# atharris/basilisk_env

Measured on AMD Instinct MI355X. Metric: env steps/sec at 65k parallel spacecraft, 1/2/4/8 MI355X; HBM GB/s vs roofline, higher is better.
Workload: dtype f64; 1 GPU; BASELINE configs[2]: 65536 envs/GPU, J2 + 4 reaction wheels (pyramid) + nadir reward, f64, dt 0.1 s, K=1 RK4 sub-step(s)/env step, FSW every 10 (fsw_lag=nav_lag=1), synthetic PCG64(rank); envs_per_gpu=65536, substeps=1, scenario=bare, batch_stats=per-wave sums in the step launch; join on demand, kernel_fingerprint=2b375b0f4a16a217

## Files before the change

basilisk_env_amd/csrc/bsk_device.hpp:

```cpp
#pragma once
#include <hip/hip_runtime.h>
#include <stdint.h>

#include <type_traits>

#include "../../include/bskgpu.h"
#include "bsk_probes.hpp"

namespace bsk {

#define BSK_LIKELY(x) __builtin_expect(!!(x), 1)
#define BSK_UNLIKELY(x) __builtin_expect(!!(x), 0)

struct V3 {
    double x, y, z;
};
__device__ __forceinline__ V3 mk(double x, double y, double z) { return V3{x, y, z}; }
__device__ __forceinline__ V3 operator+(V3 a, V3 b) { return V3{a.x + b.x, a.y + b.y, a.z + b.z}; }
__device__ __forceinline__ V3 operator-(V3 a, V3 b) { return V3{a.x - b.x, a.y - b.y, a.z - b.z}; }
__device__ __forceinline__ V3 operator*(double s, V3 a) { return V3{s * a.x, s * a.y, s * a.z}; }
__device__ __forceinline__ double dot(V3 a, V3 b) { return fma(a.x, b.x, fma(a.y, b.y, a.z * b.z)); }
__device__ __forceinline__ V3 cross(V3 a, V3 b) {
    return V3{fma(a.y, b.z, -(a.z * b.y)), fma(a.z, b.x, -(a.x * b.z)), fma(a.x, b.y, -(a.y * b.x))};
}
// ... 141 lines not shown
    double mu_sun;
    double base_density;
    double inv_scale_height, inv_mass, rho_skip;
    int32_t desat, pad_;
};

struct PowerCfg {
    double nB[3];
    double kflux;
    double draw, cap;
    double req, rs_plus, rs_minus;
    double rsun;
    double sun_r0[3], sun_v[3];
};

struct SunGeom {
    V3 sun;
    double ism;
    double re_sf1, re_sf2;
    double tf1, tf2;
};

__device__ __forceinline__ SunGeom sun_setup(const PowerCfg& pc, double t0) {
    SunGeom g;
    g.sun = mk(fma(pc.sun_v[0], t0, pc.sun_r0[0]), fma(pc.sun_v[1], t0, pc.sun_r0[1]), fma(pc.sun_v[2], t0, pc.sun_r0[2]));
    g.ism = rsqrt_nr(dot(g.sun, g.sun));
    const double sf1 = pc.rs_plus * g.ism, sf2 = pc.rs_minus * g.ism;
    g.re_sf1 = pc.req * rcp_nr(sf1);
    g.re_sf2 = pc.req * rcp_nr(sf2);
    g.tf1 = sf1 * rsqrt_nr(fma(-sf1, sf1, 1.0));
    g.tf2 = sf2 * rsqrt_nr(fma(-sf2, sf2, 1.0));
    return g;
}

__device__ __forceinline__ double asin_small(double s) {
    const double z = s * s;
    return s * fma(z, fma(z, fma(z, fma(z, 35.0 / 1152.0, 15.0 / 336.0), 3.0 / 40.0), 1.0 / 6.0), 1.0);
}

__device__ __forceinline__ double asin_core(double z) {
    double p = 0.03187962140081284;
    p = fma(p, z, -0.016187392271599134);
    p = fma(p, z, 0.019513468251252167);
    p = fma(p, z, 0.0065293020047365695);
    p = fma(p, z, 0.012170138592391726);
    p = fma(p, z, 0.01388484282640208);
    p = fma(p, z, 0.01735977964134998);
    p = fma(p, z, 0.022371749733164054);
    p = fma(p, z, 0.03038195969768514);
    p = fma(p, z, 0.044642856805998936);
    p = fma(p, z, 0.07500000000385201);
    p = fma(p, z, 0.16666666666664942);
    return fma(p, z, 1.0);
}
__device__ __forceinline__ double asin01(double s) {
    const bool big = s > 0.5;
    const double z = big ? fma(-0.5, s, 0.5) : s * s;
    const double q = big ? sqrt_nr(z) : s;
    const double r = q * asin_core(z);
    return big ? fma(-2.0, r, 1.57079632679489661923) : r;
}
__device__ __forceinline__ double angle_xy(double x, double y, double a) {
    const double ia = rcp_nr(a), t = x * ia, sy = y * ia, at = fabs(t);
    const bool big = at > 0.5;
    const double z = big ? 0.5 * sy * sy * rcp_nr(1.0 + at) : t * t;
    const double q = big ? sqrt_nr(z) : at;
    const double r = q * asin_core(z);
    const double PI = 3.14159265358979323846;
    const double base = big ? (t > 0.0 ? 0.0 : PI) : 0.5 * PI;
    const double k = big ? (t > 0.0 ? 2.0 : -2.0) : (t > 0.0 ? -1.0 : 1.0);
    return fma(k, r, base);
}

__device__ __attribute__((noinline)) double percent_shadow_generic(double sa, double sb, double cc) {
    const double PI = 3.14159265358979323846;
    const double a = asin(sa), b = asin(sb), c = acos(cc);
    if (c < a - b) return 1.0 - (b * b) / (a * a);
    const double x = (c * c + a * a - b * b) / (2.0 * c), y = sqrt(fmax(a * a - x * x, 0.0));
    const double area = a * a * acos(x / a) + b * b * acos((c - x) / b) - c * y;
    return 1.0 - area / (PI * a * a);
}

__device__ __forceinline__ double percent_shadow(const PowerCfg& pc, V3 r_HB, V3 r, double r2) {
    const double nh2 = dot(r_HB, r_HB);
    const double inh = rsqrt_nr(nh2), ins = rsqrt_nr(r2);
    const double sa = fmin(pc.rsun * inh, 1.0), sb = fmin(pc.req * ins, 1.0);
    const double cc = fmax(fmin(-dot(r, r_HB) * inh * ins, 1.0), -1.0);
    const double ca = sqrt_nr(fma(-sa, sa, 1.0)), cb = sqrt_nr(fma(-sb, sb, 1.0));
    if (sb > sa && cc > fma(cb, ca, sb * sa)) return 0.0;
    if (cc <= fma(cb, ca, -(sb * sa))) return 1.0;
    const double PI = 3.14159265358979323846;
    if (sa < 0.03125 * sb) {
        const double a = asin_small(sa), b = asin01(sb);
        const double sc = sqrt_nr(fma(-cc, cc, 1.0));
        const double d = asin_small(fma(sc, cb, -(cc * sb)));
        const double c = b + d, a2 = a * a;
        const double x = fma(d, fma(2.0, b, d), a2) * rcp_nr(2.0 * c);
        const double y = sqrt_nr(fmax(fma(-x, x, a2), 0.0));
        const double th1 = angle_xy(x, y, a);
        const double w = y * rcp_nr(b), z = w * w;
        const double t2 = w * z * fma(z, fma(z, fma(z, 35.0 / 1152.0, 15.0 / 336.0), 3.0 / 40.0), 1.0 / 6.0);
        const double area = fma(a2, th1, fma(b * b, t2, -(d * y)));
        return 1.0 - area * rcp_nr(PI * a2);
    }
    return percent_shadow_generic(sa, sb, cc);
}

constexpr int PEN_CHUNK = 10;
constexpr int PEN_SLOTS = 30;
constexpr int PEN_QCAP = 192;
struct PowerLds {
    double g[PEN_SLOTS][64];
    double s[PEN_SLOTS][64];
    double sun[3][64];
    double qr[3][PEN_QCAP];
    int qown[PEN_QCAP];
    int qcount, pad_[3];
};
typedef PowerLds __attribute__((address_space(3))) * LdsP;

constexpr int PAIR_CHUNK = 10;
struct PairLds {
    double rr[2][3][PAIR_CHUNK][64];
    double rs[2][3][PAIR_CHUNK][64];
    double box[16][64];
    double sfac[PAIR_CHUNK][64];
    double sun[3][64];
    double lext[3][64];
    int qown[PAIR_CHUNK * 64];
    int qcount, pad_[3];
};
typedef PairLds __attribute__((address_space(3))) * PairP;

constexpr int PART_ALL = 0, PART_ROT = 1, PART_TRA = 2;

constexpr int TRI_SPIN_LIMIT = 1 << 20;
enum { BSK_DEVERR_TRI_EXCHANGE = 1, BSK_DEVERR_FORK_MAP = 2 };
struct TriX {
    double v[4][4][64];
    double s[4][3][64];
    int tv[4][64], ts[4][64];
    int err, pad0_;
    int pad_[4];
};
struct TriLds {
    PairLds p;
    TriX x;
};
typedef TriX __attribute__((address_space(3))) * TriXP;
typedef TriLds __attribute__((address_space(3))) * TriP;

struct HalvesLds {
    double rv[6][64];
    unsigned long long orbit;
    unsigned long long pad_;
};
typedef HalvesLds __attribute__((address_space(3))) * HalvesP;

__device__ __forceinline__ void tri_order() { asm volatile("" ::: "memory"); }
__device__ __forceinline__ void tri_st(double __attribute__((address_space(3))) * p, double v) {
    __hip_atomic_store((long long __attribute__((address_space(3)))*)p, __double_as_longlong(v), __ATOMIC_RELAXED, __HIP_MEMORY_SCOPE_WORKGROUP);
}
__device__ __forceinline__ double tri_ld(const double __attribute__((address_space(3))) * p) {
    return __longlong_as_double(__hip_atomic_load((long long __attribute__((address_space(3)))*)p, __ATOMIC_RELAXED, __HIP_MEMORY_SCOPE_WORKGROUP));
}
__device__ __forceinline__ void tri_sti(int __attribute__((address_space(3))) * p, int v) { __hip_atomic_store(p, v, __ATOMIC_RELAXED, __HIP_MEMORY_SCOPE_WORKGROUP); }
__device__ __forceinline__ int tri_ldi(int __attribute__((address_space(3))) * p) { return __hip_atomic_load(p, __ATOMIC_RELAXED, __HIP_MEMORY_SCOPE_WORKGROUP); }

struct TriPend {
    int tag;
    V3 a;
    double e;
};
template <int PART>
struct TriXch {
    TriXP X;
    int lane;
    int np, nc;
    bool dead;
    unsigned dbg_miss = 0, dbg_spin = 0;
    unsigned long long dbg_cyc = 0;
    template <bool EXTRA>
    __device__ __forceinline__ void publish(V3 a, double extra) {
        if constexpr (probe::TRI_NOPUBLISH && PART == PART_TRA) { ++np; return; }
        const int slot = np & 3;
        if constexpr (PART == PART_TRA) {
            tri_st(&X->v[slot][0][lane], a.x); tri_st(&X->v[slot][1][lane], a.y); tri_st(&X->v[slot][2][lane], a.z);
            if constexpr (EXTRA) tri_st(&X->v[slot][3][lane], extra);
            tri_order();
            tri_sti(&X->tv[slot][lane], np + 1);
        } else {
            tri_st(&X->s[slot][0][lane], a.x); tri_st(&X->s[slot][1][lane], a.y); tri_st(&X->s[slot][2][lane], a.z);
            tri_order();
            tri_sti(&X->ts[slot][lane], np + 1);
        }
        tri_order();
        ++np;
    }
    template <bool EXTRA>
    __device__ __forceinline__ TriPend prefetch() const {
        const int slot = nc & 3;
        TriPend f;
        f.e = 0.0;
        if constexpr (PART == PART_TRA) {
            f.tag = tri_ldi(&X->ts[slot][lane]);
            tri_order();
            f.a = mk(tri_ld(&X->s[slot][0][lane]), tri_ld(&X->s[slot][1][lane]), tri_ld(&X->s[slot][2][lane]));
        } else {
            f.tag = tri_ldi(&X->tv[slot][lane]);
            tri_order();
            f.a = mk(tri_ld(&X->v[slot][0][lane]), tri_ld(&X->v[slot][1][lane]), tri_ld(&X->v[slot][2][lane]));
            if constexpr (EXTRA) f.e = tri_ld(&X->v[slot][3][lane]);
        }
        return f;
    }
    template <bool EXTRA>
    __device__ __forceinline__ V3 finish(TriPend f, double& extra) {
        const int want = nc + 1;
        if (BSK_UNLIKELY(__builtin_amdgcn_ballot_w64(f.tag != want) != 0)) {
            if constexpr (probe::XCH_STATS) ++dbg_miss;
            const probe::Stamp c0 = probe::stamp<probe::XCH_STATS>();
            for (int spin = 0; !dead; ++spin) {
                f = prefetch<EXTRA>();
                if constexpr (probe::XCH_STATS) ++dbg_spin;
                if (__builtin_amdgcn_ballot_w64(f.tag != want) == 0) break;
                if (spin > TRI_SPIN_LIMIT) { dead = true; X->err = 1; }
            }
            probe::since<probe::XCH_STATS>(dbg_cyc, c0);
        }
        ++nc;
        if constexpr (EXTRA) extra = f.e;
        return f.a;
    }
};

struct KTab {
    double a, b, c, e;
};
template <int K>
__device__ __forceinline__ double fmac_k(double acc, double tab, double x) {
    static_assert(K >= 0 && K < 16, "row lane");
    asm volatile("v_fmac_f64_dpp %0, %1, %2 row_newbcast:%3 row_mask:0xf bank_mask:0xf" : "+v"(acc) : "v"(tab), "v"(x), "n"(K));
    return acc;
}
template <int K>
__device__ __forceinline__ double fmac_k_abs(double acc, double tab, double x) {
    asm volatile("v_fmac_f64_dpp %0, %1, |%2| row_newbcast:%3 row_mask:0xf bank_mask:0xf" : "+v"(acc) : "v"(tab), "v"(x), "n"(K));
    return acc;
}
template <int K>
__device__ __forceinline__ double fmac_k_neg(double acc, double tab, double x) {
    asm volatile("v_fmac_f64_dpp %0, %1, -%2 row_newbcast:%3 row_mask:0xf bank_mask:0xf" : "+v"(acc) : "v"(tab), "v"(x), "n"(K));
    return acc;
}
__device__ __forceinline__ double max0(double x) {
    double r;
    asm("v_max_f64 %0, %1, 0" : "=v"(r) : "v"(x));
    return r;
}
template <int K>
__device__ __forceinline__ double mul_k(double tab, double x) { return fmac_k<K>(0.0, tab, x); }
template <int K>
__device__ __forceinline__ double get_k(double tab) {
    double r;
    asm volatile("v_mov_b64_dpp %0, %1 row_newbcast:%2 row_mask:0xf bank_mask:0xf" : "=v"(r) : "v"(tab), "n"(K));
    return r;
}

__device__ __forceinline__ double atmosphere_exponent(const KTab& kt, double rm) {
    return fmac_k<KC_NIH>(get_k<KC_REQIH>(kt.c), kt.c, rm);
}
__device__ __forceinline__ double atmosphere_exp(const KTab& kt, double x) {
    const double n = __builtin_rint(mul_k<KC_LOG2E>(kt.c, x));
    const double te = kt.e;
    double r = fmac_k<KE_NLN2HI>(x, te, n);
    double t0 = get_k<KE_POLY + 0>(te), t1 = get_k<KE_POLY + 2>(te), t2 = get_k<KE_POLY + 4>(te), t3 = get_k<KE_POLY + 6>(te);
    r = fmac_k<KE_NLN2LO>(r, te, n);
    double t4 = get_k<KE_POLY + 8>(te), t5 = get_k<KE_POLY + 10>(te), t6 = get_k<KE_POLY + 12>(te);
    const double r2 = r * r;
    t0 = fmac_k<KE_POLY + 1>(t0, te, r); t1 = fmac_k<KE_POLY + 3>(t1, te, r); t2 = fmac_k<KE_POLY + 5>(t2, te, r);
    t3 = fmac_k<KE_POLY + 7>(t3, te, r); t4 = fmac_k<KE_POLY + 9>(t4, te, r); t5 = fmac_k<KE_POLY + 11>(t5, te, r);
    t6 = fmac_k<KE_POLY + 13>(t6, te, r);
    double p = fma(t6, r2, t5);
    p = fma(p, r2, t4);
    p = fma(p, r2, t3);
    p = fma(p, r2, t2);
    p = fma(p, r2, t1);
    p = fma(p, r2, t0);
    return ldexp(p, (int)n);
}
struct Atmo {
    double x, rho;
    __device__ __forceinline__ double clamped(const KTab& kt) const { return rho >= get_k<KC_RSKIP>(kt.c) ? rho : 0.0; }
    __device__ __forceinline__ double anchor(const KTab& kt, double rm) {
        x = atmosphere_exponent(kt, rm);
        rho = atmosphere_exp(kt, x);
        return clamped(kt);
    }
    __device__ __forceinline__ double advance(const KTab& kt, double rm) {
        const double xn = atmosphere_exponent(kt, rm);
        const double d = xn - x;
        x = xn;
        const double d2 = d * d;
        double a = fmac_k<KC_I120>(get_k<KC_I24>(kt.c), kt.c, d);
        double b = fmac_k<KC_I6>(0.5, kt.c, d);
        a = fmac_k<KC_I720>(a, kt.c, d2);
        b = fma(d2, a, b);
// ... 995 lines not shown
```

basilisk_env_amd/csrc/bsk_kernels.hip:

```cpp
#include "bsk_device.hpp"
#include "bsk_envstep.hpp"
#include "bsk_launch.hpp"

#include <atomic>
#include <cstddef>
#define __COMMA__ ,

namespace bsk {

__device__ __forceinline__ int uni(bool b) { return __builtin_amdgcn_readfirstlane(b ? 1 : 0); }
__device__ __forceinline__ double own_scalar(double x) {
    const unsigned long long u = __builtin_bit_cast(unsigned long long, x);
    const unsigned lo = __builtin_amdgcn_readfirstlane((unsigned)u), hi = __builtin_amdgcn_readfirstlane((unsigned)(u >> 32));
    return __builtin_bit_cast(double, ((unsigned long long)hi << 32) | lo);
}
__device__ __forceinline__ int uni_any(bool lane_cond) {
    const unsigned long long m = __builtin_amdgcn_ballot_w64(lane_cond);
    int r;
    asm volatile("s_cmp_lg_u64 %1, 0\n\ts_cselect_b32 %0, 1, 0" : "=s"(r) : "s"(m) : "scc");
    return r;
}

__device__ __forceinline__ int halves_fsw_due(int cnt_x, int nav_lag, int fsw_every) {
    return uni_any((cnt_x >> 20) == (nav_lag != 0 ? fsw_every - 1 : 0));
}

__device__ __forceinline__ int wave_min_uniform(int v) {
    const int first = __builtin_amdgcn_readfirstlane(v);
    if (__builtin_amdgcn_ballot_w64(v != first) == 0) return first;
#pragma unroll
    for (int off = 32; off > 0; off >>= 1) v = min(v, __shfl_xor(v, off, 64));
    return __builtin_amdgcn_readfirstlane(v);
}

constexpr int LDSS_WAVES = 3;
template <int GRAV, int NRW, bool DIAG, int FEAT, int SPLIT>
__global__ __launch_bounds__(256, (SPLIT == 5 || SPLIT == 4 || SPLIT == 2 || SPLIT == 3 || SPLIT == 6) ? 2 : (FEAT == FEAT_LDSS ? LDSS_WAVES : 1)) void step_kernel(const StepArgs<NRW, DIAG> a) {
    const HotCfg<NRW, DIAG>& c = a.hot;
    const ColdCfg* __restrict__ cold = a.cold;
    const probe::Stamp t_kernel = probe::stamp<probe::PAIR_TIME>();
    constexpr bool TRI = SPLIT == 3;
    constexpr bool PAIR = SPLIT == 2 || TRI;
    constexpr bool HALVES = SPLIT == 6;
    const int gid = (SPLIT == 5) ? (int)(blockIdx.x * 128 + (threadIdx.x >> 7) * 64 + (threadIdx.x & 63))
                  : (PAIR || HALVES) ? (int)(blockIdx.x * 64 + (threadIdx.x & 63))
                         : (int)(blockIdx.x * blockDim.x + threadIdx.x);
    const bool valid = gid < a.n;
    const int i = valid ? gid : a.n - 1;
    const int64_t S = a.stride;
    const double* __restrict__ st = a.st;
    const uint32_t bo = (uint32_t)i * 8u;
#define FLD(f) (st + (int64_t)(f) * S)

    extern __shared__ __align__(16) unsigned char lds_dyn[];
    if constexpr (HALVES) {
        static_assert(form_built(GRAV, DIAG, FEAT, SPLIT, NRW), "the halves form: bare level, point mass or J2, with wheels (bsk_launch.hpp: form_built)");
        if (__builtin_amdgcn_readfirstlane((int)(threadIdx.x >> 6)) != 0) {
            const HalvesP HL = (HalvesP)lds_dyn;
            const int hl = (int)(threadIdx.x & 63u);
            State<NRW> xt;
            xt.r = mk(ldf(FLD(BSK_F_R + 0), bo), ldf(FLD(BSK_F_R + 1), bo), ldf(FLD(BSK_F_R + 2), bo));
            xt.v = mk(ldf(FLD(BSK_F_V + 0), bo), ldf(FLD(BSK_F_V + 1), bo), ldf(FLD(BSK_F_V + 2), bo));
            const int2 cnt_t = *reinterpret_cast<const int2*>(reinterpret_cast<const char*>(a.cnt) + bo);
            asm volatile("" ::"s"(c.h), "s"(c.h2), "s"(c.h3), "s"(c.h6), "s"(c.nmu), "s"(c.j2k));
            if (halves_fsw_due(cnt_t.x, a.nav_lag, c.fsw_every)) {
                HL->rv[0][hl] = xt.r.x; HL->rv[1][hl] = xt.r.y; HL->rv[2][hl] = xt.r.z;
                HL->rv[3][hl] = xt.v.x; HL->rv[4][hl] = xt.v.y; HL->rv[5][hl] = xt.v.z;
                __syncthreads();
            }
            const Env ev_t{};
            const WheelV<NRW> wv_t{};
            rk4_step<GRAV, NRW, DIAG, FEAT, SPLIT, false, 0, PART_TRA>(c, wv_t, xt, nullptr, mk(0, 0, 0), (double)cnt_t.y * c.h, ev_t);
            const gptr<double> so_t = uniform_ptr(a.tail.st);
            stf(so_t + (int64_t)(BSK_F_R + 0) * S, bo, xt.r.x); stf(so_t + (int64_t)(BSK_F_R + 1) * S, bo, xt.r.y);
            stf(so_t + (int64_t)(BSK_F_R + 2) * S, bo, xt.r.z);
            stf(so_t + (int64_t)(BSK_F_V + 0) * S, bo, xt.v.x); stf(so_t + (int64_t)(BSK_F_V + 1) * S, bo, xt.v.y);
            stf(so_t + (int64_t)(BSK_F_V + 2) * S, bo, xt.v.z);
            const unsigned long long below = __builtin_amdgcn_ballot_w64(dot(xt.r, xt.r) < a.tail.obs_cfg.r_min2);
            if (hl == 0) HL->orbit = below;
            __syncthreads();
            return;
        }
    }
    State<NRW> x;
    if constexpr (HALVES) {
        x.r = mk(0, 0, 0); x.v = mk(0, 0, 0);
    } else {
    x.r = mk(ldf(FLD(BSK_F_R + 0), bo), ldf(FLD(BSK_F_R + 1), bo), ldf(FLD(BSK_F_R + 2), bo));
    x.v = mk(ldf(FLD(BSK_F_V + 0), bo), ldf(FLD(BSK_F_V + 1), bo), ldf(FLD(BSK_F_V + 2), bo));
    }
    x.s = mk(ldf(FLD(BSK_F_SIGMA + 0), bo), ldf(FLD(BSK_F_SIGMA + 1), bo), ldf(FLD(BSK_F_SIGMA + 2), bo));
    x.w = mk(ldf(FLD(BSK_F_OMEGA + 0), bo), ldf(FLD(BSK_F_OMEGA + 1), bo), ldf(FLD(BSK_F_OMEGA + 2), bo));
#pragma unroll
    for (int k = 0; k < NRW; ++k) x.Om[k] = ldf(FLD(BSK_NF_BASE + k), bo);
    constexpr int TAIL = BSK_NF_BASE + NRW;
    const V3 lext = mk(ldf(FLD(TAIL + BSK_T_LEXT + 0), bo), ldf(FLD(TAIL + BSK_T_LEXT + 1), bo),
                       ldf(FLD(TAIL + BSK_T_LEXT + 2), bo));
    double charge = 1.0;
    if (FEAT >= FEAT_POWER || BSK_UNLIKELY(a.static_charge == 0)) charge = ldf(FLD(TAIL + BSK_T_CHARGE), bo);
    const int2 cnt = *reinterpret_cast<const int2*>(reinterpret_cast<const char*>(a.cnt) + bo);
    const int action = *reinterpret_cast<const int*>(reinterpret_cast<const char*>(a.act) + (bo >> a.act_shift));
    double sbr = ldf(FLD(TAIL + BSK_T_SBR), bo);
    double u[NRW > 0 ? NRW : 1], up[NRW > 0 ? NRW : 1];
#pragma unroll
    for (int k = 0; k < (NRW > 0 ? NRW : 1); ++k) up[k] = 0.0;
#pragma unroll
    for (int k = 0; k < NRW; ++k) u[k] = ldf(FLD(TAIL + BSK_T_UCMD + k), bo);
#undef FLD
    double ep_ret = 0.0;
    if (BSK_UNLIKELY(a.ep_return != nullptr)) ep_ret = ldf(a.ep_return, bo);
    asm volatile("" ::"s"(c.fsw_every), "s"(c.h), "s"(c.h2), "s"(c.h3), "s"(c.h6), "s"(c.nmu), "s"(c.j2k), "s"(c.Dm[0]), "s"(c.Dm[1]));

    constexpr bool FULL = is_full<FEAT>();
    int thr_t0 = 0, thr_cnt = 0;
    bool desat = false;
    if constexpr (FULL) desat = a.extra.desat != 0;

    const int steps0 = cnt.x & 0xFFFFF;
    int phase = cnt.x >> 20;
    bool fsw_ran = false;

    const int fsw_every = c.fsw_every;
    const int substeps = a.substeps;
    constexpr bool WDPP = FULL || (FEAT == FEAT_LDSS && NRW > 0);
    std::conditional_t<WDPP, WheelDpp<NRW, FULL>, WheelV<NRW>> wv;
    const int substeps_eff = substeps;
    int j = 0;
    int tick = cnt.y;
    bool tri_failed = false;
    double shadow = 1.0;
    SunGeom sg;
    constexpr bool POWER = FEAT >= FEAT_POWER;
    LdsP L = nullptr;
    const int lane = (int)(threadIdx.x & 63u);
    if constexpr (POWER) {
        sg = sun_setup(a.power, (double)tick * c.h);
        if constexpr (!PAIR) {
            L = (LdsP)lds_dyn + (threadIdx.x >> 6);
            L->sun[0][lane] = sg.sun.x; L->sun[1][lane] = sg.sun.y; L->sun[2][lane] = sg.sun.z;
            if (lane == 0) L->qcount = 0;
        }
    }
    AccP accp = nullptr;
    if constexpr (FEAT == FEAT_LDSS) accp = (AccP)lds_dyn + (threadIdx.x >> 6);
    KTab kt;
    if constexpr (FULL) {
        const int l16 = lane & 15;
        kt.a = cold->kt[l16]; kt.b = cold->kt[16 + l16]; kt.c = cold->kt[32 + l16]; kt.e = cold->kt[64 + l16];
        wv.ta = kt.a; wv.tb = kt.b; wv.td = cold->kt[48 + l16];
    } else if constexpr (WDPP) {
        const int l16 = lane & 15;
        wv.ta = cold->kt[l16]; wv.tb = cold->kt[16 + l16]; wv.td = cold->kt[48 + l16];
    } else {
        wv.load(c);
    }
    Env ev;
    if constexpr (FULL) {
        ev.cold = cold;
        ev.kt = kt;
        ev.sun_on = a.extra.mu_sun != 0.0;
        ev.drag_on = false;
        ev.rho = 0.0;
        ev.s3.sh = sg.ism * sg.sun;
        ev.s3.k = a.extra.mu_sun * sg.ism * sg.ism * sg.ism;
        ev.s3.A0 = mk(0, 0, 0);
        ev.thr_on = false;
        ev.e2 = 0;
        ev.m0 = ev.m1 = ev.m2 = 0;
        ev.FB0 = mk(0, 0, 0);
        ev.LB0 = mk(0, 0, 0);
        ev.facet_axis = cold->facet_axis;
#pragma unroll
        for (int k = 0; k < BSK_MAX_THR / 2; ++k) ev.thr_lim2[k] = 0u;
        ev.thr_max = 0;
        if (desat) {
#pragma unroll
            for (int k = 0; k < BSK_MAX_THR; ++k) {
                const unsigned lim = (unsigned)ldf(st + (int64_t)(TAIL + BSK_T_THR_LIM + k) * S, bo);
                ev.thr_lim2[k >> 1] |= lim << (16 * (k & 1));
                ev.thr_max = max(ev.thr_max, (int)lim);
            }
            thr_t0 = (int)ldf(st + (int64_t)(TAIL + BSK_T_THR_T0) * S, bo);
            thr_cnt = (int)ldf(st + (int64_t)(TAIL + BSK_T_THR_CNT) * S, bo);
        }
    }
    Pre pre{0.0, 0.0, MrpRot{0.0, 0.0}};
    if constexpr (FULL && !PAIR) { pre.r2 = dot(x.r, x.r); pre.rot = mrp_rot(x.s); }
    Atmo atm{0.0, 0.0};
    bool first_fsw = true;
    bool drag_cfg = false;
    if constexpr (FULL) drag_cfg = a.extra.base_density != 0.0;
    const int drag_cfg_u = uni(drag_cfg);
    bool navlag = false;
    if constexpr (NRW > 0) navlag = a.nav_lag != 0;
    double un[NRW > 0 ? NRW : 1];
#pragma unroll
    for (int k = 0; k < NRW; ++k) un[k] = u[k];
    unsigned lim2n[BSK_MAX_THR / 2] = {0u, 0u, 0u, 0u};
    int thr_maxn = 0, thr_t0n = 0;
    if constexpr (FULL) {
#pragma unroll
        for (int k = 0; k < BSK_MAX_THR / 2; ++k) lim2n[k] = ev.thr_lim2[k];
        thr_maxn = ev.thr_max;
        thr_t0n = thr_t0;
    }
    auto fsw_tick = [&](const State<NRW>& nav, int t_latch) {
        const bool lag = a.fsw_lag != 0;
        if (lag && first_fsw) {
#pragma unroll
            for (int k = 0; k < NRW; ++k) up[k] = ldf(st + (int64_t)(TAIL + BSK_T_UPEND + k) * S, bo);
        }
        const FswCfg fc = load_fsw(cold);
        Guid g = guidance<NRW>(fc.sigma_R0N, nav, action);
        sbr = sqrt_nr(dot(g.sigma_BR, g.sigma_BR));
        if (lag) {
#pragma unroll
            for (int k = 0; k < NRW; ++k) un[k] = up[k];
            control<NRW>(fc, g, up);
        } else {
            control<NRW>(fc, g, un);
        }
        fsw_ran = true;
        if constexpr (FULL) {
            if (desat && action == 2) {
                bool fired = false;
                desat_tick<NRW>(cold, nav.Om, first_fsw, fsw_every * c.h, 2.0 / c.h, fsw_every,
                                const_cast<double*>(st) + (int64_t)(TAIL + BSK_T_THR_REM) * S, S, bo, lim2n, fired, thr_cnt);
                if (fired) {
                    thr_maxn = 0;
#pragma unroll
                    for (int k = 0; k < BSK_MAX_THR; ++k) thr_maxn = max(thr_maxn, (int)((lim2n[k >> 1] >> (16 * (k & 1))) & 0xFFFFu));
                    thr_t0n = t_latch;
                }
            }
        }
        first_fsw = false;
    };
    auto latch = [&]() {
#pragma unroll
        for (int k = 0; k < NRW; ++k) u[k] = un[k];
        if constexpr (FULL) {
#pragma unroll
            for (int k = 0; k < BSK_MAX_THR / 2; ++k) ev.thr_lim2[k] = lim2n[k];
            ev.thr_max = thr_maxn;
            thr_t0 = thr_t0n;
        }
    };
    bool z0 = false;
    if constexpr (NRW > 0) z0 = navlag && tick == 0 && substeps_eff > 0;
    int since = 0;
    bool own = true;
    unsigned long long dbg_waitA = 0, dbg_waitB = 0, dbg_chain = 0, dbg_bar = 0;
    if constexpr (PAIR) {
        static_assert(form_built(GRAV, DIAG, FEAT, SPLIT), "a wave-split form this cell is not built in (bsk_launch.hpp: form_built)");
        PairP PL = (PairP)lds_dyn;
        const int wave_id = __builtin_amdgcn_readfirstlane((int)(threadIdx.x >> 6));
        const bool isD = TRI ? wave_id != 1 : ((wave_id ^ (int)(blockIdx.x >> a.pair_shift)) & 1) == 0;
        TriXP TX = nullptr;
        if constexpr (TRI) TX = (TriXP) & ((TriP)lds_dyn)->x;
        if (!isD) {
            PL->sun[0][lane] = sg.sun.x; PL->sun[1][lane] = sg.sun.y; PL->sun[2][lane] = sg.sun.z;
            PL->lext[0][lane] = lext.x; PL->lext[1][lane] = lext.y; PL->lext[2][lane] = lext.z;
            if (lane == 0) PL->qcount = 0;
// ... 407 lines not shown
                fsw_tick(nav, tick + ((navlag && !z0) ? 1 : 0));
                probe::since<probe::CHUNK == 3>(dbg_chain, pc_fsw);
                fsw_here = true;
                if (!navlag) latch();
                else dist = fsw_every;
            }
            if (anyz) dist = 0;
            z0 = false;
            m = min(m, dist);
            if constexpr (POWER) m = min(m, PEN_CHUNK);
            if constexpr (FULL) {
                own = since == 0 || fsw_here || since >= PEN_CHUNK;
                if (own) since = 0;
                m = min(m, PEN_CHUNK - since);
            }
            if constexpr (GRAV == BSK_GRAV_SH || WDPP || POWER) m = wave_min_uniform(m);
            phase += m;
            if (phase >= fsw_every) phase -= fsw_every;
        }
        if constexpr (POWER && NRW == 0) {
            m = min(m, PEN_CHUNK);
            if constexpr (FULL) m = wave_min_uniform(m);
        }
        if constexpr (POWER) {
            const probe::Stamp pc_flush = probe::stamp<probe::CHUNK == 4>();
            if (__builtin_amdgcn_ballot_w64(np + m > PEN_SLOTS) != 0) {
                power_flush(a.power, L, np, lane, c.h, charge, shadow);
                np = 0;
            }
            probe::since<probe::CHUNK == 4>(dbg_chain, pc_flush);
        }
        j += m;
        if constexpr (FULL) {
            const probe::Stamp pc_anchor = probe::stamp<probe::CHUNK == 5>();
            const V3 a0_kept = ev.s3.A0;
            const Atmo atm_kept = atm;
            if (ev.sun_on) third_body_anchor(ev.s3, sg.sun, a.extra.mu_sun, x.r);
            if (drag_cfg_u) atm.anchor(kt, pre.r2 * rsqrt_nr(pre.r2));
            if (BSK_UNLIKELY(uni_any(!own) != 0)) {
                if (!own) { ev.s3.A0 = a0_kept; atm = atm_kept; }
            }
            if constexpr (NRW > 0) since += m;
            probe::since<probe::CHUNK == 5>(dbg_chain, pc_anchor);
        }
        int burst_any = 0;
        int drag_now = 0, thr_now = 0;
        int t = 0;
        auto tick_head = [&]() __attribute__((always_inline)) {
            if constexpr (FULL) {
                pre.ir = rsqrt_nr(pre.r2);
                if (drag_cfg_u) {
                    ev.rho = atm.advance(kt, pre.r2 * pre.ir);
                    drag_now = uni_any(ev.rho != 0.0);
                }
                if (BSK_UNLIKELY(burst_any)) thr_now = uni_any(ev.thr_max > 0 && 2 * (tick - thr_t0) <= ev.thr_max);
            }
        };
        auto tick_body = [&](auto THR_, auto DM_) __attribute__((always_inline)) {
            constexpr bool THR = decltype(THR_)::value;
            constexpr int DM = decltype(DM_)::value;
            double q2 = 0.0;
            if constexpr (FULL && THR) {
                ev.e2 = 2 * (tick - thr_t0);
                ev.drag_on = drag_now != 0;
                thr_masks(ev);
            }
            if constexpr (FULL) rk4_step<GRAV, NRW, DIAG, FEAT, SPLIT, THR, DM>(c, wv, x, u, lext, (double)tick * c.h, ev, accp, &pre, &q2);
            else rk4_step<GRAV, NRW, DIAG, FEAT, SPLIT, false, 0, HALVES ? PART_ROT : PART_ALL>(c, wv, x, u, lext, (double)tick * c.h, ev, accp);
            if constexpr (POWER) power_tick<FULL>(FULL ? a.power : pc_loop_cfg, sg, x.r, x.s, L, np + t, lane, kt.c, FULL ? &pre : nullptr, FULL ? &q2 : nullptr);
            ++t;
            ++tick;
        };
        using B0 = std::integral_constant<bool, false>;
        using B1 = std::integral_constant<bool, true>;
        using I0_ = std::integral_constant<int, 0>;
        using I1_ = std::integral_constant<int, 1>;
        using I2_ = std::integral_constant<int, 2>;
        auto burst_pending = [&]() __attribute__((always_inline)) {
            int any = 0;
            if constexpr (FULL) {
                if (desat) any = uni_any(ev.thr_max > 0 && 2 * (tick - thr_t0) <= ev.thr_max);
                if (!any) thr_now = 0;
            }
            return any;
        };
        burst_any = burst_pending();
        probe::since<probe::CHUNK == 1>(dbg_chain, pc_head);
        const probe::Stamp pc_first = probe::stamp<probe::CHUNK == 2>();
        if constexpr (NRW > 0) {
            bool lat = navlag && fsw_here;
            if constexpr (GRAV == BSK_GRAV_SH || WDPP || POWER) lat = __builtin_amdgcn_ballot_w64(lat) != 0;
            if (lat && m > 0) {
                tick_head();
                if constexpr (FULL) {
                    if (BSK_LIKELY(!thr_now)) {
                        if (BSK_LIKELY(drag_now)) tick_body(B0{}, I1_{});
                        else tick_body(B0{}, I2_{});
                    } else tick_body(B1{}, I0_{});
                } else tick_body(B0{}, I0_{});
                latch();
                burst_any = burst_pending();
            }
        }
        probe::since<probe::CHUNK == 2>(dbg_chain, pc_first);
        auto run = [&](auto THR_, auto DM_) __attribute__((always_inline)) {
            constexpr bool THR = decltype(THR_)::value;
            constexpr int DM = decltype(DM_)::value;
            auto same = [&]() __attribute__((always_inline)) {
                if constexpr (!FULL) return true;
                else if constexpr (THR) return false;
                else return !thr_now && drag_now == (DM == 1 ? 1 : 0);
            };
#pragma nounroll
            for (;;) {
                tick_body(THR_, DM_);
                if (t >= m) return false;
                tick_head();
                if (BSK_UNLIKELY(!same())) return true;
                tick_body(THR_, DM_);
                if (t >= m) return false;
                tick_head();
                if (BSK_UNLIKELY(!same())) return true;
            }
        };
        if constexpr (POWER) {
            bool headed = false;
#pragma nounroll
            while (t < m) {
                if (!headed) tick_head();
                if constexpr (FULL) {
                    if (BSK_LIKELY(!thr_now)) {
                        if (BSK_LIKELY(drag_now)) headed = run(B0{}, I1_{});
                        else headed = run(B0{}, I2_{});
                    } else headed = run(B1{}, I0_{});
                } else headed = run(B0{}, I0_{});
            }
        } else {
#pragma nounroll
            while (t + 1 < m) {
                tick_body(B0{}, I0_{});
                tick_body(B0{}, I0_{});
            }
            if (t < m) tick_body(B0{}, I0_{});
        }
        np += m;
        if constexpr (NRW > 0) latch();
    }
    if constexpr (POWER) {
        if (__builtin_amdgcn_ballot_w64(np > 0) != 0) power_flush(a.power, L, np, lane, c.h, charge, shadow);
    }
    if constexpr (probe::CHUNK != 0) dbg_waitA = probe::elapsed(pc_loop);
    }

    typedef const TailArgs __attribute__((address_space(4))) * TailPtr;
    TailPtr tp = (TailPtr)((const char __attribute__((address_space(4)))*)__builtin_amdgcn_kernarg_segment_ptr() +
                           offsetof(StepArgs<NRW __COMMA__ DIAG>, tail));
    asm volatile("" : "+s"(tp));
    TailArgs ta;
    __builtin_memcpy(&ta, (const TailArgs*)tp, sizeof(TailArgs));
    const int64_t S2 = uniform64(ta.stride);
    const int64_t SO = uniform64(ta.ostride);
    const int n2 = ta.n;
    const bool valid2 = gid < n2;
    if constexpr (TRI) {
        if (BSK_UNLIKELY(tri_failed)) {
            sbr = __builtin_nan(""); charge = sbr;
            if (lane == 0) __hip_atomic_store(ta.err, BSK_DEVERR_TRI_EXCHANGE, __ATOMIC_RELAXED, __HIP_MEMORY_SCOPE_SYSTEM);
        }
    }

    double o0 = sbr;
    if (!HALVES && !(NRW > 0 && ta.nav_lag != 0)) {
        double sR0N[3] = {ta.obs_cfg.sigma_R0N[0], ta.obs_cfg.sigma_R0N[1], ta.obs_cfg.sigma_R0N[2]};
        const Guid g = guidance<NRW>(sR0N, x, action);
        o0 = sqrt_nr(dot(g.sigma_BR, g.sigma_BR));
    }
    const double o1 = sqrt_nr(dot(x.w, x.w));
    double om2 = 0.0;
#pragma unroll
    for (int k = 0; k < NRW; ++k) om2 = fma(x.Om[k], x.Om[k], om2);
    const double o2 = sqrt_nr(om2) * ta.obs_cfg.inv_wheel_limit;
    const bool static_o3 = FEAT < FEAT_POWER && ta.static_charge != 0;
    double o3 = charge * ta.obs_cfg.charge_scale;
    const double o4 = shadow;

    int why = 0;
    double rew = (action == 0) ? ta.obs_cfg.reward_mult * rcp_nr(fma(o0, o0, 1.0)) : 0.0;
    if (steps0 >= ta.obs_cfg.max_length) why |= BSK_DONE_LENGTH;
    if (o2 > 1.0) { why |= BSK_DONE_WHEELS; rew -= ta.obs_cfg.failure_penalty; }
    if (!static_o3 && o3 == 0.0) { why |= BSK_DONE_BATTERY; rew -= ta.obs_cfg.failure_penalty; }
    if constexpr (HALVES) {
        __syncthreads();
        if ((((HalvesP)lds_dyn)->orbit >> lane) & 1ull) why |= BSK_DONE_ORBIT;
    } else {
        if (dot(x.r, x.r) < ta.obs_cfg.r_min2) why |= BSK_DONE_ORBIT;
    }

    if constexpr (SPLIT == 5) {
        if (threadIdx.x & 64) return;
    }
    const unsigned long long dmask = __ballot(valid2 && why != 0);
    if constexpr (probe::ANY) {
        unsigned long long w = 0ull;
        if constexpr (TRI && probe::TRI_XCHG != 0)
            w = ((volatile unsigned long long __attribute__((address_space(3)))*)&((TriP)lds_dyn)->x.pad_[0])[probe::TRI_XCHG == 2 ? 1 : 0];
        if constexpr (PAIR && probe::PAIR_WAIT)
            w = ((dbg_waitB >> 4) & 0x1FFFFFull) | (((dbg_waitA >> 4) & 0x1FFFFFull) << 21) | (((unsigned long long)((PairP)lds_dyn)->box[10][0] & 0x1FFFFFull) << 42);
        if constexpr (PAIR && probe::PAIR_TIME)
            w = ((probe::elapsed(t_kernel) >> 10) & 0xFFFFFFFFull) | (probe::hw_id() << 32);
        if constexpr (PAIR && probe::PAIR_HWID)
            w = probe::hw_id() | ((unsigned long long)((PairP)lds_dyn)->box[9][0] << 32);
        if constexpr (!PAIR && probe::CHUNK != 0)
            w = ((dbg_chain >> 4) & 0xFFFFFFFFull) | (((dbg_waitA >> 4) & 0xFFFFFFFFull) << 32);
        if ((threadIdx.x & 63) == 0 && ta.dbg && !(TRI && probe::TRI_ROLE)) ta.dbg[gid >> 6] = w;
    }
    if ((threadIdx.x & 63) == 0) {
        ta.done_mask[gid >> 6] = dmask;
    }

    gptr<double> so = uniform_ptr(ta.st);
    gptr<double> ob = uniform_ptr(ta.obs);
#define FLD(f) (so + (int64_t)(f) * S2)
    const int n_pool = HALVES ? 0 : ta.n_pool;
    if (n_pool > 0 && why != 0) {
      if (valid2) {
        gptr<double> tob = uniform_ptr(ta.term_obs);
        if (static_o3) o3 = *(gptr<double>)((gptr<char>)(ob + 3 * SO) + bo);
        stf(tob + 0 * SO, bo, o0); stf(tob + 1 * SO, bo, o1); stf(tob + 2 * SO, bo, o2); stf(tob + 3 * SO, bo, o3);
        stf(tob + 4 * SO, bo, o4);
        const int ep = ta.episodes[i];
        ta.episodes[i] = ep + 1;
        const unsigned slot = pool_slot((unsigned)i + ta.env_base, (unsigned)ep, (unsigned)n_pool);
        const double* __restrict__ pool = ta.pool;
        const int nf = ta.n_fields;
        for (int f = 0; f < nf; ++f) stf(FLD(f), bo, pool[(int64_t)f * n_pool + slot]);
        const V3 ps = mk(pool[(int64_t)(BSK_F_SIGMA + 0) * n_pool + slot], pool[(int64_t)(BSK_F_SIGMA + 1) * n_pool + slot],
                         pool[(int64_t)(BSK_F_SIGMA + 2) * n_pool + slot]);
        const V3 pw = mk(pool[(int64_t)(BSK_F_OMEGA + 0) * n_pool + slot], pool[(int64_t)(BSK_F_OMEGA + 1) * n_pool + slot],
                         pool[(int64_t)(BSK_F_OMEGA + 2) * n_pool + slot]);
        double pom2 = 0.0;
#pragma unroll
        for (int k = 0; k < NRW; ++k) {
            const double v = pool[(int64_t)(BSK_NF_BASE + k) * n_pool + slot];
            pom2 = fma(v, v, pom2);
        }
        const Obs5 f0 = first_observation(ps, pw, pom2, pool[(int64_t)(TAIL + BSK_T_CHARGE) * n_pool + slot], ta.obs_cfg.inv_wheel_limit,
                                          ta.obs_cfg.charge_scale);
        stf(ob + 0 * SO, bo, f0.o[0]); stf(ob + 1 * SO, bo, f0.o[1]); stf(ob + 2 * SO, bo, f0.o[2]); stf(ob + 3 * SO, bo, f0.o[3]);
        stf(ob + 4 * SO, bo, f0.o[4]);
        if (ta.obs_rm) {
            double* __restrict__ rm = ta.obs_rm + (int64_t)i * 5;
            rm[0] = f0.o[0]; rm[1] = f0.o[1]; rm[2] = f0.o[2]; rm[3] = f0.o[3]; rm[4] = f0.o[4];
        }
        *(gptr<unsigned long long>)((gptr<char>)uniform_ptr(ta.cnt) + bo) = 0ull;
      }
    } else {
        if constexpr (!HALVES) {
        stf(FLD(BSK_F_R + 0), bo, x.r.x); stf(FLD(BSK_F_R + 1), bo, x.r.y); stf(FLD(BSK_F_R + 2), bo, x.r.z);
        stf(FLD(BSK_F_V + 0), bo, x.v.x); stf(FLD(BSK_F_V + 1), bo, x.v.y); stf(FLD(BSK_F_V + 2), bo, x.v.z);
        }
        stf(FLD(BSK_F_SIGMA + 0), bo, x.s.x); stf(FLD(BSK_F_SIGMA + 1), bo, x.s.y); stf(FLD(BSK_F_SIGMA + 2), bo, x.s.z);
        stf(FLD(BSK_F_OMEGA + 0), bo, x.w.x); stf(FLD(BSK_F_OMEGA + 1), bo, x.w.y); stf(FLD(BSK_F_OMEGA + 2), bo, x.w.z);
#pragma unroll
        for (int k = 0; k < NRW; ++k) stf(FLD(BSK_NF_BASE + k), bo, x.Om[k]);
        if constexpr (POWER) stf(FLD(TAIL + BSK_T_CHARGE), bo, charge);
        if constexpr (FULL) {
            if (desat) {
#pragma unroll
                for (int k = 0; k < BSK_MAX_THR; ++k) stf(FLD(TAIL + BSK_T_THR_LIM + k), bo, (double)thr_limit(ev, k));
                stf(FLD(TAIL + BSK_T_THR_T0), bo, (double)thr_t0);
                stf(FLD(TAIL + BSK_T_THR_CNT), bo, (double)thr_cnt);
            }
        }
        if constexpr (NRW > 0) {
            if (fsw_ran) {
#pragma unroll
                for (int k = 0; k < NRW; ++k) stf(FLD(TAIL + BSK_T_UCMD + k), bo, u[k]);
                if (ta.fsw_lag) {
#pragma unroll
                    for (int k = 0; k < NRW; ++k) stf(FLD(TAIL + BSK_T_UPEND + k), bo, up[k]);
                }
                stf(FLD(TAIL + BSK_T_SBR), bo, sbr);
            }
        }
        const unsigned long long packed = (unsigned long long)(unsigned)(min(steps0 + 1, 0xFFFFF) | (phase << 20)) |
                                          ((unsigned long long)(unsigned)(cnt.y + ta.substeps) << 32);
        *(gptr<unsigned long long>)((gptr<char>)uniform_ptr(ta.cnt) + bo) = packed;
        stf(ob + 0 * SO, bo, o0); stf(ob + 1 * SO, bo, o1); stf(ob + 2 * SO, bo, o2);
        if (!static_o3) stf(ob + 3 * SO, bo, o3);
        stf(ob + 4 * SO, bo, o4);
        if (ta.obs_rm) {
            double* __restrict__ rm = ta.obs_rm + (int64_t)i * 5;
            rm[0] = o0; rm[1] = o1; rm[2] = o2; rm[4] = o4;
            if (!static_o3) rm[3] = o3;
        }
    }
#undef FLD
    stf(uniform_ptr(ta.reward), bo, rew);
    ta.reason[i] = (unsigned char)why;
    if (ta.ep_return) {
        ep_ret += rew;
        if (why != 0) {
            stf(uniform_ptr(ta.term_return), bo, ep_ret);
            ta.term_len[i] = steps0;
            if (n_pool > 0) ep_ret = 0.0;
        }
        stf(uniform_ptr(ta.ep_return), bo, ep_ret);
        ta.done[i] = why != 0 ? 1 : 0;
    }
    if (BSK_UNLIKELY(ta.wave_sum != nullptr)) {
        const double ws = wave_sum(valid2 ? rew : 0.0);
        if ((threadIdx.x & 63) == 0) ta.wave_sum[gid >> 6] = ws;
    }
}

template <int GRAV, int NRW, bool DIAG, int FEAT, int SPLIT>
static hipError_t launch_t(const StepLaunch& go, const LaunchShape& sh) {
    const StepParams& p = go.p;
    const StepBuffers& b = go.b;
    StepArgs<NRW, DIAG> a;
    fill_hot<GRAV, NRW, DIAG>(p, a.hot);
    a.cold = b.cold; a.st = b.tail.st; a.cnt = b.tail.cnt; a.act = b.act;
    a.stride = b.tail.stride; a.n = b.tail.n; a.substeps = b.tail.substeps;
    a.nav_lag = p.nav_lag; a.fsw_lag = p.fsw_lag;
    a.pair_shift = p.pair_shift; a.act_shift = b.act_shift; a.ep_return = b.tail.ep_return;
    a.static_charge = b.tail.static_charge; a.pad2_ = 0;
    a.power = p.pc;
    a.extra = p.ex;
    a.tail = b.tail;
    if (sh.lds > 48 * 1024) {
        static std::atomic<unsigned long long> raised{0ull};
        int dev = 0;
        hipError_t e = hipGetDevice(&dev);
        if (e != hipSuccess) return e;
        const unsigned long long bit = 1ull << (dev & 63);
        if (!(raised.load(std::memory_order_acquire) & bit)) {
            e = hipFuncSetAttribute((const void*)&step_kernel<GRAV, NRW, DIAG, FEAT, SPLIT>,
                                    hipFuncAttributeMaxDynamicSharedMemorySize, (int)sh.lds);
            if (e != hipSuccess) return e;
            raised.fetch_or(bit, std::memory_order_release);
        }
    }
    hipExtLaunchKernelGGL((step_kernel<GRAV, NRW, DIAG, FEAT, SPLIT>), dim3(sh.grid), dim3(sh.block), sh.lds, go.s, go.ev0, go.ev1, 0, a);
    return hipGetLastError();
}

#define BSK_CELL(X, G, D, P) X(G, 0, D, P) X(G, 3, D, P) X(G, 4, D, P)
#define BSK_UNIT0(X) BSK_CELL(X, BSK_GRAV_SH, true, 3)
#define BSK_UNIT1(X) BSK_CELL(X, BSK_GRAV_SH, true, 2)
#define BSK_UNIT2(X) BSK_CELL(X, BSK_GRAV_SH, false, 3)
#define BSK_UNIT3(X) BSK_CELL(X, BSK_GRAV_SH, false, 2)
#define BSK_UNIT4(X) BSK_CELL(X, BSK_GRAV_SH, true, 0) BSK_CELL(X, BSK_GRAV_SH, true, 1) BSK_CELL(X, BSK_GRAV_SH, false, 0)
#define BSK_UNIT5(X) BSK_CELL(X, BSK_GRAV_SH, false, 1) BSK_CELL(X, BSK_GRAV_PM, true, 2) BSK_CELL(X, BSK_GRAV_PM_J2, true, 2)
#define BSK_UNIT6(X) BSK_CELL(X, BSK_GRAV_PM_J2, true, 0) BSK_CELL(X, BSK_GRAV_PM_J2, true, 1) BSK_CELL(X, BSK_GRAV_PM_J2, true, 3)   \
                   BSK_CELL(X, BSK_GRAV_PM_J2, false, 0) BSK_CELL(X, BSK_GRAV_PM_J2, false, 1) BSK_CELL(X, BSK_GRAV_PM_J2, false, 2) \
                   BSK_CELL(X, BSK_GRAV_PM_J2, false, 3) BSK_CELL(X, BSK_GRAV_PM_J2, true, -1) BSK_CELL(X, BSK_GRAV_PM_J2, false, -1)
#define BSK_UNIT7(X) BSK_CELL(X, BSK_GRAV_PM, true, 0) BSK_CELL(X, BSK_GRAV_PM, true, 1) BSK_CELL(X, BSK_GRAV_PM, true, 3)            \
                   BSK_CELL(X, BSK_GRAV_PM, false, 0) BSK_CELL(X, BSK_GRAV_PM, false, 1) BSK_CELL(X, BSK_GRAV_PM, false, 2)          \
                   BSK_CELL(X, BSK_GRAV_PM, false, 3) BSK_CELL(X, BSK_GRAV_PM, true, -1) BSK_CELL(X, BSK_GRAV_PM, false, -1)
#if defined(BSK_TU)
#define BSK_TU_CAT2(a, b) a##b
#define BSK_TU_CAT(a, b) BSK_TU_CAT2(a, b)
#define BSK_VARIANTS(X) BSK_TU_CAT(BSK_UNIT, BSK_TU)(X)
#define BSK_STEP_UNIT BSK_TU_CAT(dispatch_step_tu, BSK_TU)
#else
#define BSK_STEP_UNIT dispatch_step
#if defined(BSK_ONLY)
#define BSK_VARIANTS(X) BSK_ONLY(X)
#elif defined(BSK_FAST_BUILD) && BSK_FAST_BUILD == 3
#define BSK_VARIANTS(X) X(BSK_GRAV_PM_J2, 3, true, 2)
#elif defined(BSK_FAST_BUILD) && BSK_FAST_BUILD == 2
#define BSK_VARIANTS(X) X(BSK_GRAV_SH, 4, true, 0) X(BSK_GRAV_SH, 4, true, 1) X(BSK_GRAV_SH, 4, true, 2) X(BSK_GRAV_SH, 4, true, 3)
#elif defined(BSK_FAST_BUILD)
#define BSK_FAST_LEVELS(X, R) X(BSK_GRAV_PM_J2, R, true, 0) X(BSK_GRAV_PM_J2, R, true, 1) X(BSK_GRAV_PM_J2, R, true, 2) X(BSK_GRAV_PM_J2, R, true, 3) X(BSK_GRAV_PM_J2, R, true, -1)
#define BSK_VARIANTS(X) BSK_FAST_LEVELS(X, 4) BSK_FAST_LEVELS(X, 3)
#else
#define BSK_VARIANTS(X) BSK_UNIT0(X) BSK_UNIT1(X) BSK_UNIT2(X) BSK_UNIT3(X) BSK_UNIT4(X) BSK_UNIT5(X) BSK_UNIT6(X) BSK_UNIT7(X)
#endif
#endif

template <int G, int R, bool D, int P, int S>
static hipError_t step_form(int block, int n, const StepLaunch* go, KernelDesc* d) {
    if constexpr (form_built(G, D, P, S, R)) {
        d->fn = (const void*)&step_kernel<G, R, D, P, S>;
        d->shape = launch_shape(S, P, block, n);
        return go ? launch_t<G, R, D, P, S>(*go, d->shape) : hipSuccess;
    } else {
        return hipErrorInvalidValue;
    }
}

hipError_t BSK_STEP_UNIT(int grav, int nrw, bool diag, int feat, int form, int block, int n, const StepLaunch* go, KernelDesc* d) {
#define CASE(G, R, D, P, S) \
    if (grav == G && nrw == R && diag == D && feat == P && form == S) return step_form<G, R, D, P, S>(block, n, go, d);
#define SPLIT_FORMS(G, R, D, P) CASE(G, R, D, P, FORM_TRI) CASE(G, R, D, P, FORM_PAIR)
#define ONE_WAVE_FORMS(G, R, D, P) CASE(G, R, D, P, FORM_SH_DPP) CASE(G, R, D, P, FORM_SH_DPP2) CASE(G, R, D, P, FORM_SINGLE)
    BSK_VARIANTS(SPLIT_FORMS)
    BSK_VARIANTS(ONE_WAVE_FORMS)
#define HALVES_FORM(G, R, D, P) CASE(G, R, D, P, FORM_HALVES)
    BSK_VARIANTS(HALVES_FORM)
#undef HALVES_FORM
#undef ONE_WAVE_FORMS
#undef SPLIT_FORMS
#undef CASE
    return hipErrorInvalidValue;
}

}
```

Baseline: 11.14 billion env-steps/s.

## Move halves-form step epilogue (obs, reward, done, counters) onto the translation wave

In the halves split, the attitude wave now only writes its attitude and wheel state plus three per-lane quantities (omega squared, wheel speed squared, sbr) into LDS, then returns. The translation wave reads these after the barrier and does the observations, reward, termination reasons, done mask, counter packing, episode return and wave sums. The aim is to shorten the attitude wave's critical path by handing it work the lighter orbit wave can absorb. The cost is more LDS traffic and a dropped pool-reset path for HALVES, and termination and reset semantics now depend on the moved epilogue being correct.

```diff
diff --git a/basilisk_env_amd/csrc/bsk_device.hpp b/basilisk_env_amd/csrc/bsk_device.hpp
--- a/basilisk_env_amd/csrc/bsk_device.hpp
+++ b/basilisk_env_amd/csrc/bsk_device.hpp
@@ -317,7 +317,8 @@
 
 struct HalvesLds {
     double rv[6][64];
-    unsigned long long orbit;
+    double hand[3][64];
+    unsigned long long dbg;
     unsigned long long pad_;
 };
 typedef HalvesLds __attribute__((address_space(3))) * HalvesP;
diff --git a/basilisk_env_amd/csrc/bsk_kernels.hip b/basilisk_env_amd/csrc/bsk_kernels.hip
--- a/basilisk_env_amd/csrc/bsk_kernels.hip
+++ b/basilisk_env_amd/csrc/bsk_kernels.hip
@@ -23,6 +23,30 @@
 
 __device__ __forceinline__ int halves_fsw_due(int cnt_x, int nav_lag, int fsw_every) {
     return uni_any((cnt_x >> 20) == (nav_lag != 0 ? fsw_every - 1 : 0));
+}
+
+__device__ __forceinline__ int halves_phase_after(int cnt_x, int fsw_every) {
+    const int phase = (cnt_x >> 20) + 1;
+    return phase >= fsw_every ? phase - fsw_every : phase;
+}
+
+#define BSK_STEP_OUTCOME(oc, action, steps0, o0, o2, o3, static_o3, r2)                                   \
+    int why = 0;                                                                                          \
+    double rew = ((action) == 0) ? (oc).reward_mult * rcp_nr(fma((o0), (o0), 1.0)) : 0.0;                 \
+    if ((steps0) >= (oc).max_length) why |= BSK_DONE_LENGTH;                                              \
+    if ((o2) > 1.0) { why |= BSK_DONE_WHEELS; rew -= (oc).failure_penalty; }                              \
+    if (!(static_o3) && (o3) == 0.0) { why |= BSK_DONE_BATTERY; rew -= (oc).failure_penalty; }            \
+    if ((r2) < (oc).r_min2) why |= BSK_DONE_ORBIT
+
+template <int NRW, bool DIAG>
+__device__ __forceinline__ TailArgs load_tail() {
+    typedef const TailArgs __attribute__((address_space(4))) * TailPtr;
+    TailPtr tp = (TailPtr)((const char __attribute__((address_space(4)))*)__builtin_amdgcn_kernarg_segment_ptr() +
+                           offsetof(StepArgs<NRW __COMMA__ DIAG>, tail));
+    asm volatile("" : "+s"(tp));
+    TailArgs ta;
+    __builtin_memcpy(&ta, (const TailArgs*)tp, sizeof(TailArgs));
+    return ta;
 }
 
 __device__ __forceinline__ int wave_min_uniform(int v) {
@@ -62,6 +86,12 @@
             xt.r = mk(ldf(FLD(BSK_F_R + 0), bo), ldf(FLD(BSK_F_R + 1), bo), ldf(FLD(BSK_F_R + 2), bo));
             xt.v = mk(ldf(FLD(BSK_F_V + 0), bo), ldf(FLD(BSK_F_V + 1), bo), ldf(FLD(BSK_F_V + 2), bo));
             const int2 cnt_t = *reinterpret_cast<const int2*>(reinterpret_cast<const char*>(a.cnt) + bo);
+            const int action_t = *reinterpret_cast<const int*>(reinterpret_cast<const char*>(a.act) + (bo >> a.act_shift));
+            double charge_t = 1.0;
+            if (BSK_UNLIKELY(a.static_charge == 0)) charge_t = ldf(FLD(BSK_NF_BASE + NRW + BSK_T_CHARGE), bo);
+            double ep_ret_t = 0.0;
+            if (BSK_UNLIKELY(a.ep_return != nullptr)) ep_ret_t = ldf(a.ep_return, bo);
+            const TailArgs ta = load_tail<NRW, DIAG>();
             asm volatile("" ::"s"(c.h), "s"(c.h2), "s"(c.h3), "s"(c.h6), "s"(c.nmu), "s"(c.j2k));
             if (halves_fsw_due(cnt_t.x, a.nav_lag, c.fsw_every)) {
                 HL->rv[0][hl] = xt.r.x; HL->rv[1][hl] = xt.r.y; HL->rv[2][hl] = xt.r.z;
@@ -71,14 +101,57 @@
             const Env ev_t{};
             const WheelV<NRW> wv_t{};
             rk4_step<GRAV, NRW, DIAG, FEAT, SPLIT, false, 0, PART_TRA>(c, wv_t, xt, nullptr, mk(0, 0, 0), (double)cnt_t.y * c.h, ev_t);
-            const gptr<double> so_t = uniform_ptr(a.tail.st);
+            const gptr<double> so_t = uniform_ptr(ta.st);
             stf(so_t + (int64_t)(BSK_F_R + 0) * S, bo, xt.r.x); stf(so_t + (int64_t)(BSK_F_R + 1) * S, bo, xt.r.y);
             stf(so_t + (int64_t)(BSK_F_R + 2) * S, bo, xt.r.z);
             stf(so_t + (int64_t)(BSK_F_V + 0) * S, bo, xt.v.x); stf(so_t + (int64_t)(BSK_F_V + 1) * S, bo, xt.v.y);
             stf(so_t + (int64_t)(BSK_F_V + 2) * S, bo, xt.v.z);
-            const unsigned long long below = __builtin_amdgcn_ballot_w64(dot(xt.r, xt.r) < a.tail.obs_cfg.r_min2);
-            if (hl == 0) HL->orbit = below;
+            const double r2_t = dot(xt.r, xt.r);
+            const int64_t SO = uniform64(ta.ostride);
+            const int steps0 = cnt_t.x & 0xFFFFF;
+            const unsigned long long packed = (unsigned long long)(unsigned)(min(steps0 + 1, 0xFFFFF) | (halves_phase_after(cnt_t.x, c.fsw_every) << 20)) |
+                                              ((unsigned long long)(unsigned)(cnt_t.y + ta.substeps) << 32);
+            const bool static_o3 = ta.static_charge != 0;
+            const double o3 = charge_t * ta.obs_cfg.charge_scale;
+            const gptr<double> ob = uniform_ptr(ta.obs), ob1 = ob + SO, ob2 = ob + 2 * SO, ob3 = ob + 3 * SO, ob4 = ob + 4 * SO;
+            asm volatile("" ::"v"(r2_t), "v"(packed), "v"(o3), "v"(steps0), "s"(ob1), "s"(ob2), "s"(ob3), "s"(ob4));
             __syncthreads();
+            const double o0 = HL->hand[2][hl];
+            const double o1 = sqrt_nr(HL->hand[0][hl]);
+            const double o2 = sqrt_nr(HL->hand[1][hl]) * ta.obs_cfg.inv_wheel_limit;
+            const double o4 = 1.0;
+            BSK_STEP_OUTCOME(ta.obs_cfg, action_t, steps0, o0, o2, o3, static_o3, r2_t);
+            const unsigned long long dmask = __ballot(valid && why != 0);
+            if (hl == 0) {
+                if constexpr (probe::CHUNK != 0) {
+                    if (ta.dbg) ta.dbg[gid >> 6] = HL->dbg;
+                }
+                ta.done_mask[gid >> 6] = dmask;
+            }
+            *(gptr<unsigned long long>)((gptr<char>)uniform_ptr(ta.cnt) + bo) = packed;
+            stf(ob, bo, o0); stf(ob1, bo, o1); stf(ob2, bo, o2);
+            if (!static_o3) stf(ob3, bo, o3);
+            stf(ob4, bo, o4);
+            if (ta.obs_rm) {
+                double* __restrict__ rm = ta.obs_rm + (int64_t)i * 5;
+                rm[0] = o0; rm[1] = o1; rm[2] = o2; rm[4] = o4;
+                if (!static_o3) rm[3] = o3;
+            }
+            stf(uniform_ptr(ta.reward), bo, rew);
+            ta.reason[i] = (unsigned char)why;
+            if (ta.ep_return) {
+                ep_ret_t += rew;
+                if (why != 0) {
+                    stf(uniform_ptr(ta.term_return), bo, ep_ret_t);
+                    ta.term_len[i] = steps0;
+                }
+                stf(uniform_ptr(ta.ep_return), bo, ep_ret_t);
+                ta.done[i] = why != 0 ? 1 : 0;
+            }
+            if (BSK_UNLIKELY(ta.wave_sum != nullptr)) {
+                const double ws = wave_sum(valid ? rew : 0.0);
+                if (hl == 0) ta.wave_sum[gid >> 6] = ws;
+            }
             return;
         }
     }
@@ -97,7 +170,9 @@
     const V3 lext = mk(ldf(FLD(TAIL + BSK_T_LEXT + 0), bo), ldf(FLD(TAIL + BSK_T_LEXT + 1), bo),
                        ldf(FLD(TAIL + BSK_T_LEXT + 2), bo));
     double charge = 1.0;
+    if constexpr (!HALVES) {
     if (FEAT >= FEAT_POWER || BSK_UNLIKELY(a.static_charge == 0)) charge = ldf(FLD(TAIL + BSK_T_CHARGE), bo);
+    }
     const int2 cnt = *reinterpret_cast<const int2*>(reinterpret_cast<const char*>(a.cnt) + bo);
     const int action = *reinterpret_cast<const int*>(reinterpret_cast<const char*>(a.act) + (bo >> a.act_shift));
     double sbr = ldf(FLD(TAIL + BSK_T_SBR), bo);
@@ -108,7 +183,9 @@
     for (int k = 0; k < NRW; ++k) u[k] = ldf(FLD(TAIL + BSK_T_UCMD + k), bo);
 #undef FLD
     double ep_ret = 0.0;
+    if constexpr (!HALVES) {
     if (BSK_UNLIKELY(a.ep_return != nullptr)) ep_ret = ldf(a.ep_return, bo);
+    }
     asm volatile("" ::"s"(c.fsw_every), "s"(c.h), "s"(c.h2), "s"(c.h3), "s"(c.h6), "s"(c.nmu), "s"(c.j2k), "s"(c.Dm[0]), "s"(c.Dm[1]));
 
     constexpr bool FULL = is_full<FEAT>();
@@ -822,12 +899,37 @@
     if constexpr (probe::CHUNK != 0) dbg_waitA = probe::elapsed(pc_loop);
     }
 
-    typedef const TailArgs __attribute__((address_space(4))) * TailPtr;
-    TailPtr tp = (TailPtr)((const char __attribute__((address_space(4)))*)__builtin_amdgcn_kernarg_segment_ptr() +
-                           offsetof(StepArgs<NRW __COMMA__ DIAG>, tail));
-    asm volatile("" : "+s"(tp));
-    TailArgs ta;
-    __builtin_memcpy(&ta, (const TailArgs*)tp, sizeof(TailArgs));
+    if constexpr (HALVES) {
+        const HalvesP HL = (HalvesP)lds_dyn;
+        HL->hand[0][lane] = dot(x.w, x.w);
+        double om2 = 0.0;
+#pragma unroll
+        for (int k = 0; k < NRW; ++k) om2 = fma(x.Om[k], x.Om[k], om2);
+        HL->hand[1][lane] = om2;
+        HL->hand[2][lane] = sbr;
+        if constexpr (probe::CHUNK != 0) {
+            if (lane == 0) HL->dbg = ((dbg_chain >> 4) & 0xFFFFFFFFull) | (((dbg_waitA >> 4) & 0xFFFFFFFFull) << 32);
+        }
+        __syncthreads();
+        const gptr<double> so = uniform_ptr(const_cast<double*>(st));
+        stf(so + (int64_t)(BSK_F_SIGMA + 0) * S, bo, x.s.x); stf(so + (int64_t)(BSK_F_SIGMA + 1) * S, bo, x.s.y);
+        stf(so + (int64_t)(BSK_F_SIGMA + 2) * S, bo, x.s.z);
+        stf(so + (int64_t)(BSK_F_OMEGA + 0) * S, bo, x.w.x); stf(so + (int64_t)(BSK_F_OMEGA + 1) * S, bo, x.w.y);
+        stf(so + (int64_t)(BSK_F_OMEGA + 2) * S, bo, x.w.z);
+#pragma unroll
+        for (int k = 0; k < NRW; ++k) stf(so + (int64_t)(BSK_NF_BASE + k) * S, bo, x.Om[k]);
+        if (fsw_ran) {
+#pragma unroll
+            for (int k = 0; k < NRW; ++k) stf(so + (int64_t)(TAIL + BSK_T_UCMD + k) * S, bo, u[k]);
+            if (a.fsw_lag) {
+#pragma unroll
+                for (int k = 0; k < NRW; ++k) stf(so + (int64_t)(TAIL + BSK_T_UPEND + k) * S, bo, up[k]);
+            }
+            stf(so + (int64_t)(TAIL + BSK_T_SBR) * S, bo, sbr);
+        }
+        return;
+    }
+    const TailArgs ta = load_tail<NRW, DIAG>();
     const int64_t S2 = uniform64(ta.stride);
     const int64_t SO = uniform64(ta.ostride);
     const int n2 = ta.n;
@@ -840,7 +942,7 @@
     }
 
     double o0 = sbr;
-    if (!HALVES && !(NRW > 0 && ta.nav_lag != 0)) {
+    if (!(NRW > 0 && ta.nav_lag != 0)) {
         double sR0N[3] = {ta.obs_cfg.sigma_R0N[0], ta.obs_cfg.sigma_R0N[1], ta.obs_cfg.sigma_R0N[2]};
         const Guid g = guidance<NRW>(sR0N, x, action);
         o0 = sqrt_nr(dot(g.sigma_BR, g.sigma_BR));
@@ -854,17 +956,7 @@
     double o3 = charge * ta.obs_cfg.charge_scale;
     const double o4 = shadow;
 
-    int why = 0;
-    double rew = (action == 0) ? ta.obs_cfg.reward_mult * rcp_nr(fma(o0, o0, 1.0)) : 0.0;
-    if (steps0 >= ta.obs_cfg.max_length) why |= BSK_DONE_LENGTH;
-    if (o2 > 1.0) { why |= BSK_DONE_WHEELS; rew -= ta.obs_cfg.failure_penalty; }
-    if (!static_o3 && o3 == 0.0) { why |= BSK_DONE_BATTERY; rew -= ta.obs_cfg.failure_penalty; }
-    if constexpr (HALVES) {
-        __syncthreads();
-        if ((((HalvesP)lds_dyn)->orbit >> lane) & 1ull) why |= BSK_DONE_ORBIT;
-    } else {
-        if (dot(x.r, x.r) < ta.obs_cfg.r_min2) why |= BSK_DONE_ORBIT;
-    }
+    BSK_STEP_OUTCOME(ta.obs_cfg, action, steps0, o0, o2, o3, static_o3, dot(x.r, x.r));
 
     if constexpr (SPLIT == 5) {
         if (threadIdx.x & 64) return;
@@ -891,7 +983,7 @@
     gptr<double> so = uniform_ptr(ta.st);
     gptr<double> ob = uniform_ptr(ta.obs);
 #define FLD(f) (so + (int64_t)(f) * S2)
-    const int n_pool = HALVES ? 0 : ta.n_pool;
+    const int n_pool = ta.n_pool;
     if (n_pool > 0 && why != 0) {
       if (valid2) {
         gptr<double> tob = uniform_ptr(ta.term_obs);
@@ -925,10 +1017,8 @@
         *(gptr<unsigned long long>)((gptr<char>)uniform_ptr(ta.cnt) + bo) = 0ull;
       }
     } else {
-        if constexpr (!HALVES) {
         stf(FLD(BSK_F_R + 0), bo, x.r.x); stf(FLD(BSK_F_R + 1), bo, x.r.y); stf(FLD(BSK_F_R + 2), bo, x.r.z);
         stf(FLD(BSK_F_V + 0), bo, x.v.x); stf(FLD(BSK_F_V + 1), bo, x.v.y); stf(FLD(BSK_F_V + 2), bo, x.v.z);
-        }
         stf(FLD(BSK_F_SIGMA + 0), bo, x.s.x); stf(FLD(BSK_F_SIGMA + 1), bo, x.s.y); stf(FLD(BSK_F_SIGMA + 2), bo, x.s.z);
         stf(FLD(BSK_F_OMEGA + 0), bo, x.w.x); stf(FLD(BSK_F_OMEGA + 1), bo, x.w.y); stf(FLD(BSK_F_OMEGA + 2), bo, x.w.z);
 #pragma unroll
```

Measured after the change: 12.09 billion env-steps/s, median of 6. 1.09x the previous value.
